# UoB-HPC/neutral

Measured on AMD Instinct MI355X. Metric: particle-steps/sec, higher is better.
Workload: dtype f64

## Files before the change

neutral_amd/csrc/neutral_abi.hip:

```cpp
#include "neutral_abi_state.h"

#include <utility>

using namespace neutral_abi;


namespace {

struct StageMs {
  double kernel = 0.0, sort = 0.0, stream = 0.0, collide = 0.0, exported = 0.0, exchange = 0.0;
};

struct Step {
  neutral::SolveArgs a = {};
  neutral::StepOptions options;
  bool tiled = false;
  bool decomposed = false;
  bool exchange = false;
  bool pass_export = false;
  bool checked = false;
  State::Store* shard = nullptr;
  neutral::StepCounters hc[2] = {};
  unsigned long long check[8] = {0};
  unsigned ctrl[16] = {0};
  unsigned long long words[kStepWords] = {0};
  int passes = 0;
  int attempts = 0;
  int same = 0;
  unsigned long long queue_total = 0;
  uint64_t local_nprocessed = 0;
  StageMs stage;
};

struct BatchSpec {
  neutral::TiledPlan plan;
  int first_pass;
  bool first_sort_timed;
  bool guarded;
  const neutral::SplitExport* split;
};

BatchSpec first_batch(const neutral::SplitExport* split) {
  BatchSpec spec = {};
  spec.plan.stream_passes = g.plan_passes > 0 ? g.plan_passes + 1 : 2;
  spec.plan.blocks_per_cu = -1;
  spec.first_pass = 0;
  spec.first_sort_timed = true;
  spec.guarded = true;
  spec.split = split;
  return spec;
}

BatchSpec later_batch(int stream_passes, int first_pass) {
  BatchSpec spec = {};
  spec.plan.stream_passes = stream_passes;
  spec.plan.blocks_per_cu = -1;
  spec.first_pass = first_pass;
  return spec;
}

void harvest(Step& s, bool with_sort) {
  StageMs& stage = s.stage;
  float ms = 0.0f;
  HIP_CHECK(hipEventElapsedTime(&ms, g.ev_start, g.ev_stop));
  stage.kernel += (double)ms;
  if (s.tiled) {
    if (with_sort) {
      HIP_CHECK(hipEventElapsedTime(&ms, g.ev_start, g.ev_sorted));
      stage.sort += (double)ms;
      HIP_CHECK(hipEventElapsedTime(&ms, g.ev_sorted, g.ev_streamed));
    } else {
      HIP_CHECK(hipEventElapsedTime(&ms, g.ev_start, g.ev_streamed));
    }
    stage.stream += (double)ms;
    HIP_CHECK(hipEventElapsedTime(&ms, g.ev_streamed, g.ev_collected));
    stage.sort += (double)ms;
    HIP_CHECK(hipEventElapsedTime(&ms, g.ev_collected, g.ev_stop));
    stage.collide += (double)ms;
  } else {
    stage.collide += (double)ms;
  }
  HIP_CHECK(hipEventElapsedTime(&ms, g.ev_stop, g.ev_exported));
  stage.exported += (double)ms;
  if (s.exchange) {
    HIP_CHECK(hipEventElapsedTime(&ms, g.ev_exchange_begins, g.ev_exchanged));
    stage.exchange += (double)ms;
  }
}

void export_records_by_id(const Step& s, const int* abort_flag) {
  const neutral::SolveArgs& a = s.a;
  HIP_CHECK(neutral::launch_export_records(
      g.tiled.rec_out, g.tiled.slot_of_id, a.p, a.nparticles, g.stream, abort_flag,
      a.export_skip_long_dead ? neutral::tiled_first_inactive(g.tiled) : nullptr, 0xFFFFFFFFu,
      nullptr, 0, a.export_skip_long_dead != 0));
}

void run_batch(Step& s, const BatchSpec& spec) {
  neutral::SolveArgs& a = s.a;
  HIP_CHECK(hipEventRecord(g.ev_start, g.stream));
  if (s.tiled) {
    HIP_CHECK(neutral::launch_solve_tiled(a, s.options, g.tiled, g.stream, spec.plan, spec.first_pass,
                                          spec.first_sort_timed ? g.ev_sorted : nullptr, g.ev_streamed,
                                          g.ev_collected, &s.passes, spec.split));
  } else {
    HIP_CHECK(neutral::launch_solve(a, s.options, g.variant, g.stream));
  }
  HIP_CHECK(hipEventRecord(g.ev_stop, g.stream));
  if (s.exchange) {
    exchange_step(a, s.tiled);
  } else {
    tallies_to_caller(a);
  }
  if (spec.split) {
    HIP_CHECK(neutral::launch_split_export(a, g.tiled, *spec.split, g.ev_collected));
    HIP_CHECK(hipStreamWaitEvent(g.stream, g.ev_split_done, 0));
  } else if (s.pass_export && !s.decomposed) {
    export_records_by_id(s, spec.guarded ? a.abort_flag : nullptr);
  }
  HIP_CHECK(hipEventRecord(g.ev_exported, g.stream));
  a.export_view = nullptr;
  g.tiled.mark_suspended = 0;

  if (s.exchange) {
    finish_exchange();
  }
  publish_results(s.tiled, s.exchange);
  wait_for_stream();
// ... 658 lines not shown
```

neutral_amd/csrc/neutral_abi_state.h:

```cpp
#ifndef NEUTRAL_AMD_ABI_STATE_H
#define NEUTRAL_AMD_ABI_STATE_H

#include "../../include/neutral_hip.h"

#include <hip/hip_runtime.h>

#include <math.h>
#include <stdio.h>
#include <stdlib.h>
#include <string.h>

#include "neutral_comm.h"
#include "neutral_kernels.h"

extern "C" {
#include "../host/comms.h"
}

extern "C" {
int get_key_value_parameter(const char* specifier, const char* filename, char* keys,
                            double* values, int* nkeys);
int within_tolerance(const double expected, const double result, const double tolerance);
}

// ... 81 lines not shown
  bool use_checked = false;
  const void* checked_density = nullptr;
  bool said_checked = false;
  unsigned short* d_index[2] = {nullptr, nullptr};
  unsigned short* d_index_fine = nullptr;
  hipEvent_t ev_start = nullptr;
  hipEvent_t ev_stop = nullptr;
  hipEvent_t ev_sorted = nullptr;
  hipEvent_t ev_streamed = nullptr;
  hipEvent_t ev_collected = nullptr;
  hipEvent_t ev_exported = nullptr;
  struct StepResults* h_results = nullptr;
  struct StepResults* d_results = nullptr;
  hipStream_t comm_stream = nullptr;
  hipEvent_t ev_exchanged = nullptr;
  hipEvent_t ev_exchange_begins = nullptr;
  TableView tables;
  neutral::TiledArgs tiled = {};
  const void* rec_owner = nullptr;
  neutral::ParticleView rec_owner_view = {};
  int rec_count = 0;
  bool rec_valid = false;
  bool carried_valid = false;
  bool soa_valid = true;
  int lazy_export = 0;
  int plan_passes = 0;
  unsigned final_from = 0xFFFFFFFFu;
  int host_syncs = 0;
  int exchange_rounds = 0;
  unsigned long long emigrants = 0;
  int host_collectives = 0;
  unsigned long long* d_words = nullptr;
  MeshTally tallies[kMeshTallies] = {{1, 0, false}, {1, 0, false}, {2, 0, true}, {2, 1, true}, {4, 1, true}};
  double* d_susp_current = nullptr;
  size_t susp_current_particles = 0;
  double roulette_cutoff = 0.0;
  double roulette_survival = 0.0;
  double* d_step_scalars = nullptr;
  double* spectrum_out = nullptr;
  int spectrum_ngroups = 0;
  int spectrum_box[4] = {0, 0, 0, 0};
  double spectrum_edges[neutral::kSpectrumMaxGroups + 1] = {};
  int auto_shard = 1;
  struct Store {
    const void* key;
    int count;
    uint64_t first;
    bool decomposed;
    int capacity;
    unsigned* keys;
  };
  bool domain_on = false;
  neutral::DomainGrid domain = {1, 1, 0, 0};
  double source_box[4] = {0.0, 0.0, 0.0, 0.0};
  bool source_box_set = false;
  unsigned* d_exchange = nullptr;
  neutral::ParticleRec* d_send = nullptr;
  neutral::ParticleRec* d_recv = nullptr;
  size_t send_capacity = 0;
  size_t recv_capacity = 0;
  unsigned* rec_owner_keys = nullptr;
  unsigned* d_free_slots = nullptr;
  size_t free_slots_capacity = 0;
  int free_count = 0;
  enum { kMaxStores = 64 };
  Store stores[kMaxStores] = {};
  int nstores = 0;
  double mesh_width = 1.0;
  double mesh_height = 1.0;
  const void* extent_edges = nullptr;
  double edge_dx = 0.0;
  double edge_dy = 0.0;
  int extent_nx = 0;
  int extent_ny = 0;
  int tiled_particles = 0;
  int tiled_tiles = 0;
  int tiled_chunks = 0;
  hipStream_t export_stream = nullptr;
  hipEvent_t ev_split_done = nullptr;
  neutral::ParticleView* d_export_view = nullptr;
  neutral::ParticleView h_export_view = {};
  bool export_view_uploaded = false;
  double suspended_share = -1.0;
  size_t susp_id_words = 0;
  neutral::LaunchTuning tuning = {};
  bool tuning_read = false;
  void* d_comb = nullptr;
  size_t comb_bytes = 0;
  int stream_queues = 0;
  size_t queue_places = 0;
  int queue_tiles = 0;
};

extern State g;

enum StepWord : int {
  kWordCounters = 0,
  kWordRequeued = 8,
  kWordCollidePasses = 9,
  kWordTurnedDown = 10,
  kWordMigrants = 11,
  kWordQueued = 12,
  kWordAborted = 13,
  kWordRanks = 14,
  kWordSteals = 15,
  kWordStealsRefused = 16,
  kWordWeightedWaves = 17,
  kWordRouletteKilled = 18,
  kWordRouletteSurvived = 19,
  kStepWords = 20,
};

void ensure_scratch();
void read_variant_env();
void wait_for_stream();
void* device_zalloc(size_t bytes);
void sync_soa();
void drop_records();
void ensure_tiled_workspace(int nx, int ny, int nparticles_now, int capacity);
void before_device_write(const void* dst, size_t bytes);
void refresh_table_view(const NeutralHipCrossSection* cs_s, const NeutralHipCrossSection* cs_a,
                        bool force, bool fast_arithmetic);
neutral::ParticleView view_of(const NeutralHipParticle* p);
const State::Store* find_store(const NeutralHipParticle* p);
State::Store* remember_store(const NeutralHipParticle* p, int count, uint64_t first);
void forget_store(const NeutralHipParticle* p);
inline bool flux_code_on() {
  return g.tallies[kTallyFlux].caller[0] != nullptr || g.tallies[kTallyCurrent].caller[0] != nullptr ||
         g.tallies[kTallyOutflow].caller[0] != nullptr;
}
neutral::StepOptions begin_step_scoring(neutral::SolveArgs& a, double* energy_tally, bool tiled,
                                        bool exchange);
void run_inject(const int nparticles, const int local_nx, const int local_ny, const int pad,
                const double left_off, const double bottom_off, const double width,
                const double height, const int x_off, const int y_off, const double dt,
                const double* edgex, const double* edgey, const double initial_energy,
                const NeutralHipParticle* particles);
void run_inject_filtered(State::Store* st, const int nparticles, const int local_nx,
                         const int local_ny, const int pad, const double left_off,
                         const double bottom_off, const double width, const double height,
                         const int x_off, const int y_off, const double dt, const double* edgex,
                         const double* edgey, const double initial_energy,
                         const NeutralHipParticle* particles);

void exchange_step(const neutral::SolveArgs& a, bool tiled);
void tallies_to_caller(const neutral::SolveArgs& a);
void finish_exchange();
void publish_results(bool tiled, bool with_words);
void fetch_results(neutral::StepCounters* hc, unsigned long long* check, unsigned* ctrl,
                   unsigned long long* words);
int exchange_particles(const neutral::SolveArgs& a, neutral::TiledArgs& t);

}
#endif
```

neutral_amd/csrc/neutral_abi_store.hip:

```cpp
#include "neutral_abi_state.h"

namespace neutral_abi {

State g;


void ensure_scratch() {
  int dev = 0;
  HIP_CHECK(hipGetDevice(&dev));
  if (g.scratch_device == dev) {
    return;
  }
  HIP_CHECK(hipMalloc((void**)&g.d_counters, 2 * sizeof(neutral::StepCounters)));
  HIP_CHECK(hipMalloc((void**)&g.d_check, 16 * sizeof(unsigned long long)));
  HIP_CHECK(hipMemset(g.d_check, 0, 16 * sizeof(unsigned long long)));
  HIP_CHECK(hipMalloc((void**)&g.d_exchange, sizeof(unsigned) * 200));
  HIP_CHECK(hipMalloc((void**)&g.d_words, sizeof(unsigned long long) * kStepWords));
  HIP_CHECK(hipMalloc((void**)&g.d_step_scalars, kStepScalars * sizeof(double)));
  g.tables.valid = false;
  HIP_CHECK(hipMalloc((void**)&g.d_index_fine,
                      sizeof(unsigned short) * (kMaxFineIndexBuckets + 1)));
  for (unsigned short*& d : g.d_index) {
    HIP_CHECK(hipMalloc((void**)&d, sizeof(unsigned short) * (kMaxIndexBuckets + 1)));
  }
  HIP_CHECK(hipEventCreate(&g.ev_start));
  HIP_CHECK(hipEventCreate(&g.ev_stop));
  HIP_CHECK(hipEventCreate(&g.ev_sorted));
  HIP_CHECK(hipEventCreate(&g.ev_streamed));
  HIP_CHECK(hipEventCreate(&g.ev_collected));
  HIP_CHECK(hipEventCreate(&g.ev_exported));
  HIP_CHECK(hipEventCreate(&g.ev_exchanged));
  HIP_CHECK(hipEventCreate(&g.ev_exchange_begins));
  HIP_CHECK(hipStreamCreateWithFlags(&g.comm_stream, hipStreamNonBlocking));
  {
    int least = 0, greatest = 0;
    HIP_CHECK(hipDeviceGetStreamPriorityRange(&least, &greatest));
    HIP_CHECK(hipStreamCreateWithPriority(&g.export_stream, hipStreamNonBlocking, least));
    HIP_CHECK(hipEventCreateWithFlags(&g.ev_split_done, hipEventDisableTiming));
    HIP_CHECK(hipMalloc((void**)&g.d_export_view, sizeof(neutral::ParticleView)));
    g.export_view_uploaded = false;
  }
  if (!g.h_results) {
    HIP_CHECK(hipHostMalloc((void**)&g.h_results, sizeof(StepResults), hipHostMallocMapped));
    memset(g.h_results, 0, sizeof(StepResults));
  }
  HIP_CHECK(hipHostGetDevicePointer((void**)&g.d_results, g.h_results, 0));
  g.scratch_device = dev;
}

void read_variant_env() {
  if (!g.variant_from_env_done) {
    g.variant_from_env_done = true;
    const char* v = getenv("NEUTRAL_HIP_VARIANT");
    if (v && *v) {
      const int iv = atoi(v);
      if (iv == NEUTRAL_HIP_VARIANT_OVER_PARTICLE || iv == NEUTRAL_HIP_VARIANT_EVENT_SORTED ||
          iv == NEUTRAL_HIP_VARIANT_TILED) {
        g.variant = iv;
      } else {
        fprintf(stderr, "libneutral_hip: ignoring NEUTRAL_HIP_VARIANT=%s\n", v);
      }
    }
  }
  if (!g.arithmetic_from_env_done) {
    g.arithmetic_from_env_done = true;
    const char* arith = getenv("NEUTRAL_HIP_ARITH");
    if (arith && strcmp(arith, "checked") == 0) {
      g.arithmetic = NEUTRAL_HIP_ARITH_CHECKED;
    }
  }
}

void wait_for_stream() {
  HIP_CHECK(hipStreamSynchronize(g.stream));
  g.host_syncs++;
}

void* device_zalloc(size_t bytes) {
  void* p = nullptr;
  HIP_CHECK(hipMalloc(&p, bytes ? bytes : 1));
  HIP_CHECK(hipMemsetAsync(p, 0, bytes ? bytes : 1, g.stream));
  HIP_CHECK(hipStreamSynchronize(g.stream));
  return p;
}

neutral::CsIndex build_index(const double* d_keys, int n, unsigned short* d_start,
                             int first_shift = 44 ,
                             int max_buckets = kMaxIndexBuckets) {
  neutral::CsIndex ix = {nullptr, 0, 0, 0};
  if (n < 2 || n > 65535) {
    return ix;
  }
  double ends[2];
  HIP_CHECK(hipMemcpyAsync(&ends[0], d_keys, sizeof(double), hipMemcpyDeviceToHost, g.stream));
  HIP_CHECK(hipMemcpyAsync(&ends[1], d_keys + (n - 1), sizeof(double), hipMemcpyDeviceToHost,
                           g.stream));
  wait_for_stream();
  if (!(ends[0] > 0.0) || !(ends[1] > ends[0])) {
    return ix;
  }
  long long lo_bits, hi_bits;
  memcpy(&lo_bits, &ends[0], sizeof(lo_bits));
  memcpy(&hi_bits, &ends[1], sizeof(hi_bits));
  int shift = first_shift;
  while (((hi_bits >> shift) - (lo_bits >> shift) + 1) > max_buckets) {
    shift++;
  }
  ix.shift = shift;
  ix.base = lo_bits >> shift;
  ix.nbuckets = (int)((hi_bits >> shift) - ix.base + 1);
  HIP_CHECK(neutral::launch_build_cs_index(d_keys, n, ix.shift, ix.base, ix.nbuckets, d_start,
                                           g.stream));
  ix.start = d_start;
  return ix;
}

void sync_soa() {
  if (!g.soa_valid && g.rec_valid && g.rec_owner) {
    if (g.rec_owner_keys) {
      HIP_CHECK(neutral::launch_export_by_slot(g.tiled.rec_in, g.rec_owner_view, g.rec_owner_keys,
                                               g.rec_count, g.stream));
    } else {
      HIP_CHECK(neutral::launch_export_records(g.tiled.rec_in, g.tiled.slot_of_id,
// ... 856 lines not shown
```

neutral_amd/csrc/neutral_kernels.h:

```cpp
#ifndef NEUTRAL_AMD_KERNELS_H
#define NEUTRAL_AMD_KERNELS_H

#include <hip/hip_runtime.h>
#include <stdint.h>

namespace neutral {

struct ParticleView {
  double* x;
  double* y;
  double* omega_x;
  double* omega_y;
  double* energy;
  double* weight;
  double* dt_to_census;
  double* mfp_to_collision;
  int* cellx;
  int* celly;
  int* dead;
};

struct alignas(16) ParticleRec {
  double x, y, dt_to_census, mfp_to_collision;
  int cellx, celly;
// ... 116 lines not shown
  CarriedStart* carried;
  int steal_min;
  StealWork* steal;
  int steal_delay;
  int occupancy_rows;
  int share_weight;
  int weighted_share_min;
  int compute_units;
  int export_skip_long_dead;
  const ParticleView* export_view;
  int decomposed;
  unsigned* emigrants;
  const int* abort_flag;
};

struct TiledArgs {
  ParticleRec* rec_in;
  ParticleRec* rec_out;
  unsigned* info_in;
  unsigned* info_out;
  unsigned* id_in;
  unsigned* id_out;
  unsigned* slot_of_id;
  CarriedStart* carried_in;
  CarriedStart* carried_out;
  int carried;
  int sort_end;
  int mirror_end;
  int slots_by_id;
  unsigned* order;
  unsigned* tile_count;
  unsigned* tile_offset;
  unsigned* tile_cursor;
  uint4* chunks;
  unsigned* collide_queue;
  unsigned* susp_ids;
  int mark_suspended;
  SuspendExtra* susp;
  double* susp_track;
  StealWork* steal;
  unsigned* queue_entries;
  unsigned* queue_tail;
  unsigned* queue_head;
  unsigned queue_capacity;
  const unsigned short* fine_index;
  int fine_index_n;
  long long fine_index_base;
  int fine_index_shift;
  int* edges_computed;
  unsigned char* tile_uniform;
  unsigned* ctrl;
  int chunk_particles;
  int refill_min;
  int stream_repeat;
  int pass;
  int allow_migrate;
  double cells_per_x;
  double cells_per_y;
  int tile_shift;
  int window_min_particles;
  int tiles_x;
  int tiles_y;
  int ntiles;
  int reach_classes;
  int nsort;
  int max_chunks;
};

struct LaunchTuning {
  int steal_min;
  int share_weight;
  int weighted_share_min;
  int steal_delay;
  int max_blocks;
  int compute_units;
};
LaunchTuning launch_tuning_from_env();

struct DomainGrid {
  int px, py;
  int bx, by;
};

struct TiledPlan {
  int stream_passes;
  int blocks_per_cu;
};

enum Variant {
  kVariantOverParticle = 0,
  kVariantEventSorted = 1,
  kVariantTiled = 2,
};

hipError_t launch_inject(const InjectArgs& a, hipStream_t stream);
hipError_t launch_inject_filtered(const InjectArgs& a, unsigned* keys, unsigned* count,
                                  hipStream_t stream);
constexpr int kSpectrumMaxGroups = 64;
struct SpectrumParams {
  double* buffer;
  int ngroups;
  int x0, y0;
  unsigned width, height;
  double edges[kSpectrumMaxGroups + 1];
};
struct CurrentParams {
  double* jx;
  double* jy;
  double* susp;
};
struct StepOptions {
  double* collision_tallies = nullptr;
  double roulette_cutoff = 0.0;
  double roulette_survival = 0.0;
  SpectrumParams spectrum = {};
  CurrentParams current = {nullptr, nullptr, nullptr};
  double* outflow = nullptr;
};
enum Score : unsigned {
  kScoreCollisions = 1,
  kScoreRoulette = 2,
  kScoreSpectrum = 4,
  kScoreCurrent = 8,
  kScoreOutflow = 16,
};
constexpr int kScoreBits = 5;
constexpr unsigned kScoresOfStreaming = kScoreSpectrum | kScoreCurrent | kScoreOutflow;
inline unsigned scores_of(const StepOptions& o) {
  return (o.collision_tallies ? kScoreCollisions : 0u) | (o.roulette_cutoff > 0.0 ? kScoreRoulette : 0u) |
         (o.spectrum.ngroups > 0 ? kScoreSpectrum : 0u) | (o.current.jx ? kScoreCurrent : 0u) |
         (o.outflow ? kScoreOutflow : 0u);
}
constexpr bool scores_instantiated(bool flux, unsigned scores) {
  return flux || !(scores & (kScoreCurrent | kScoreOutflow));
}
hipError_t set_step_options(const StepOptions& o, hipStream_t stream);
hipError_t set_step_options_tiled(const StepOptions& o, hipStream_t stream);
hipError_t launch_solve(const SolveArgs& a, const StepOptions& o, int variant, hipStream_t stream);
hipError_t launch_unphysical_values(const double* v, long long n, unsigned long long* out,
                                    hipStream_t stream);
hipError_t launch_tables_check(const double* ks, const double* vs, int ns, const double* ka,
                               const double* va, int na, unsigned long long expect_hash_s,
                               unsigned long long expect_hash_a, int expect_same,
                               int fast_arithmetic, unsigned long long* out4,
                               hipStream_t stream);


size_t tiled_lds_bytes(const SolveArgs& a, const StepOptions& o, const TiledArgs& t);
hipError_t launch_import_records(const ParticleView& p, ParticleRec* rec, unsigned* info,
                                 unsigned* slot_of_id, unsigned* ids, int tiles_x, int tile_shift,
                                 int x_off, int y_off, int n, hipStream_t stream);
hipError_t launch_refresh_micro(const SolveArgs& a, const TiledArgs& t, hipStream_t stream);
bool tiled_uses_carried(const SolveArgs& a, const TiledArgs& t);
hipError_t launch_export_records(const ParticleRec* rec, const unsigned* slot_of_id,
                                 const ParticleView& p, int n, hipStream_t stream,
                                 const int* abort_flag = nullptr,
                                 const unsigned* first_inactive = nullptr,
                                 unsigned final_from = 0xFFFFFFFFu,
                                 const unsigned* skip_ids = nullptr, int max_blocks = 0,
                                 bool partial_ok = false);
struct SplitExport {
  bool on;
  hipStream_t side;
  hipEvent_t done;
  ParticleView p;
  int skip_long_dead;
};
// ... 65 lines not shown
```

neutral_amd/csrc/neutral_tiled.hip:

```cpp
#include <cstdlib>
#include <cstring>
#include <type_traits>

#include "neutral_kernels.h"

#include "neutral_device.h"
#include "neutral_history.h"
#include "neutral_step_options.h"
#include "neutral_wave.h"

namespace neutral {

#ifndef NEUTRAL_STREAM_BLOCK
#define NEUTRAL_STREAM_BLOCK 1024
#endif
constexpr int kStreamBlock = NEUTRAL_STREAM_BLOCK;
constexpr int kChunkParticlesMax = 32768;
constexpr int kChunkParticlesMin = 1024;
constexpr int kStreamRefillMin = 56;
constexpr int kStreamRepeat = 64;
constexpr int kStreamRepeatOnePass = 128;
#ifdef NEUTRAL_NO_CARRIED_START
constexpr bool kCarriedStart = false;
#else
// ... 54 lines not shown
__device__ __forceinline__ bool step_is_broken(const SolveArgs& a) {
  return a.counters->aborted != 0u;
}

__global__ __launch_bounds__(kSortBlock) void tile_count_kernel(SolveArgs a, TiledArgs t) {
  extern __shared__ unsigned s_bins[];
  if (pass_is_empty(t) || (t.pass > 0 && step_is_broken(a))) {
    return;
  }
  const int nbins = t.nsort + 1;
  const bool in_lds = nbins <= kSortLdsBins;
  if (in_lds) {
    for (int b = threadIdx.x; b < nbins; b += kSortBlock) {
      s_bins[b] = 0;
    }
    __syncthreads();
  }
  const unsigned* info = sort_summaries(t);
  const long long base = (long long)blockIdx.x * kSortSegment;
#pragma unroll 4
  for (int k = 0; k < kSortItems; ++k) {
    const long long i = base + (long long)k * kSortBlock + threadIdx.x;
    const unsigned b = (i < t.sort_end) ? sort_bucket(t, info[i]) : kNoBucket;
    if (in_lds) {
      if (b != kNoBucket) {
        atomicAdd(&s_bins[b], 1u);
      }
    } else {
      const bool is_dead = (b == (unsigned)t.nsort);
      const unsigned long long m_dead = __ballot(is_dead);
      if (b != kNoBucket && !is_dead) {
        atomicAdd(&t.tile_count[b], 1u);
      }
      if (m_dead != 0 && (threadIdx.x & 63) == (unsigned)__ffsll((long long)m_dead) - 1u) {
        atomicAdd(&t.tile_count[t.nsort], (unsigned)__popcll(m_dead));
      }
    }
  }
  if (in_lds) {
    __syncthreads();
    for (int b = threadIdx.x; b < nbins; b += kSortBlock) {
      const unsigned c = s_bins[b];
      if (c) {
        atomicAdd(&t.tile_count[b], c);
      }
    }
  }
}

__global__ __launch_bounds__(1024) void tile_scan_kernel(TiledArgs t) {
  __shared__ unsigned s_part[1024];
  const int tid = threadIdx.x;
  const int n = t.nsort + 2;
  const int per = (n + 1023) / 1024;
  const int lo = (tid * per < n) ? tid * per : n;
  const int hi = (lo + per < n) ? lo + per : n;
  unsigned sum = 0;
  for (int i = lo; i < hi; ++i) {
    sum += (i <= t.nsort) ? t.tile_count[i] : 0u;
  }
  s_part[tid] = sum;
  __syncthreads();
  for (int off = 1; off < 1024; off <<= 1) {
    const unsigned c0 = (tid >= off) ? s_part[tid - off] : 0;
    __syncthreads();
    s_part[tid] += c0;
    __syncthreads();
  }
  if (tid == 0) {
    t.ctrl[kCtrlWindowed] = 0;
  }
  unsigned run = s_part[tid] - sum;
  for (int i = lo; i < hi; ++i) {
    const unsigned c = (i <= t.nsort) ? t.tile_count[i] : 0u;
    t.tile_offset[i] = run;
    t.tile_cursor[i] = run;
    if (i <= t.nsort) {
      t.tile_count[i] = 0;
    }
    run += c;
  }
}

__device__ __forceinline__ void draw_for_slot(const SolveArgs& a, const TiledArgs& t, long long slot) {
  t.carried_in[slot].minus_log_rn0 = draw_first_flight(a.pid_base + (uint64_t)t.id_in[slot], a.master_key);
}

__global__ __launch_bounds__(kSortBlock) void tile_scatter_kernel(SolveArgs a, TiledArgs t) {
  extern __shared__ unsigned s_bins[];
  if (pass_is_empty(t) || (t.pass > 0 && step_is_broken(a))) {
    return;
  }
  const bool draws = t.pass == 0 && t.carried != 0;
  const int nbins = t.nsort + 1;
  const bool in_lds = nbins <= kSortLdsBins;
  unsigned* s_rank = s_bins;
  unsigned* s_base = s_bins + nbins;
  const unsigned* info = sort_summaries(t);
  const long long base = (long long)blockIdx.x * kSortSegment;
  unsigned bucket[kSortItems];
#pragma unroll
  for (int k = 0; k < kSortItems; ++k) {
    const long long i = base + (long long)k * kSortBlock + threadIdx.x;
    bucket[k] = (i < t.sort_end) ? sort_bucket(t, info[i]) : kNoBucket;
  }
  if (!in_lds) {
#pragma unroll
    for (int k = 0; k < kSortItems; ++k) {
      const bool is_dead = (bucket[k] == (unsigned)t.nsort);
      const unsigned long long m_dead = __ballot(is_dead);
      unsigned dead_base = 0;
      if (m_dead != 0) {
        const unsigned leader = (unsigned)__ffsll((long long)m_dead) - 1u;
        if ((threadIdx.x & 63) == leader) {
          dead_base = atomicAdd(&t.tile_cursor[t.nsort], (unsigned)__popcll(m_dead));
        }
        dead_base = __shfl(dead_base, (int)leader, 64);
      }
      if (bucket[k] != kNoBucket) {
        const unsigned pos = is_dead ? dead_base + (unsigned)lane_rank(m_dead)
                                     : atomicAdd(&t.tile_cursor[bucket[k]], 1u);
        t.order[pos] = (unsigned)(base + (long long)k * kSortBlock + threadIdx.x);
        if (draws && !is_dead) {
          draw_for_slot(a, t, base + (long long)k * kSortBlock + threadIdx.x);
        }
      }
    }
    return;
  }
  for (int b = threadIdx.x; b < nbins; b += kSortBlock) {
    s_rank[b] = 0;
  }
  __syncthreads();
#pragma unroll
  for (int k = 0; k < kSortItems; ++k) {
    if (bucket[k] != kNoBucket) {
      atomicAdd(&s_rank[bucket[k]], 1u);
    }
  }
  __syncthreads();
  for (int b = threadIdx.x; b < nbins; b += kSortBlock) {
    const unsigned c = s_rank[b];
    if (c) {
      s_base[b] = atomicAdd(&t.tile_cursor[b], c);
      s_rank[b] = 0;
    }
  }
  __syncthreads();
#pragma unroll
  for (int k = 0; k < kSortItems; ++k) {
    if (bucket[k] != kNoBucket) {
      const unsigned pos = s_base[bucket[k]] + atomicAdd(&s_rank[bucket[k]], 1u);
      t.order[pos] = (unsigned)(base + (long long)k * kSortBlock + threadIdx.x);
    }
  }
  if (draws) {
#pragma unroll 1
    for (int k = 0; k < kSortItems; ++k) {
      if (bucket[k] != kNoBucket && bucket[k] != (unsigned)t.nsort) {
        draw_for_slot(a, t, base + (long long)k * kSortBlock + threadIdx.x);
      }
    }
  }
}

__global__ __launch_bounds__(kSortBlock) void copy_inactive_kernel(SolveArgs a, TiledArgs t) {
  if (a.abort_flag && *a.abort_flag) {
    return;
  }
  const unsigned first_inactive = t.tile_offset[t.nsort];
  const unsigned ncarried = (unsigned)t.sort_end - first_inactive;
  const unsigned total = ncarried + (unsigned)(t.mirror_end - t.sort_end);
  for (unsigned u = blockIdx.x * kSortBlock + threadIdx.x; u < total; u += gridDim.x * kSortBlock) {
  if (u < ncarried) {
    const unsigned j = first_inactive + u;
    const unsigned src = t.order[j];
    const ParticleRec r = t.rec_in[src];
    t.rec_out[j] = r;
    t.info_out[j] = t.info_in[src];
    if (a.decomposed) {
      t.id_out[j] = t.id_in[src];
    } else {
      t.slot_of_id[r.id] = j;
    }
  } else {
    const unsigned m = (unsigned)t.sort_end + (u - ncarried);
    if (m < (unsigned)t.mirror_end) {
      t.rec_out[m] = t.rec_in[m];
      t.info_out[m] = t.info_in[m];
    }
  }
  }
}

__global__ __launch_bounds__(kSortBlock) void collect_suspended_kernel(SolveArgs a, TiledArgs t,
                                                                       const unsigned* info) {
  __shared__ unsigned s_count[kSortItems][kSortBlock / 64];
  __shared__ unsigned s_base;
  if (step_is_broken(a)) {
    return;
  }
  const long long base = (long long)blockIdx.x * kSortSegment;
  const int wave = threadIdx.x >> 6;
  unsigned mine = 0;
#pragma unroll
  for (int k = 0; k < kSortItems; ++k) {
    const long long i = base + (long long)k * kSortBlock + threadIdx.x;
    const bool susp = i < t.sort_end && summary_state(info[i]) == kRecCollide;
    const unsigned long long m = __ballot(susp);
    mine |= susp ? (1u << k) : 0u;
    if ((threadIdx.x & 63) == 0) {
      s_count[k][wave] = (unsigned)__popcll(m);
    }
  }
  __syncthreads();
  if (threadIdx.x == 0) {
    unsigned total = 0;
    for (int k = 0; k < kSortItems; ++k) {
      for (int w = 0; w < kSortBlock / 64; ++w) {
        const unsigned c = s_count[k][w];
        s_count[k][w] = total;
        total += c;
      }
    }
    s_base = total ? atomicAdd(&t.ctrl[kCtrlCollideCount], total) : 0u;
  }
  __syncthreads();
  if (mine) {
#pragma unroll
    for (int k = 0; k < kSortItems; ++k) {
      const bool susp = ((mine >> k) & 1u) != 0;
      const unsigned long long m = __ballot(susp);
      if (susp) {
        const unsigned slot = (unsigned)(base + (long long)k * kSortBlock + threadIdx.x);
        t.collide_queue[s_base + s_count[k][wave] + (unsigned)lane_rank(m)] = slot;
        if (t.mark_suspended) {
          const unsigned id = t.rec_out[slot].id;
          atomicOr(&t.susp_ids[id >> 5], 1u << (id & 31u));
        }
      }
    }
  }
}

__global__ __launch_bounds__(kSortBlock) void import_records_kernel(ParticleView p, ParticleRec* rec,
                                                                    unsigned* info,
// ... 1125 lines not shown
         kStreamLdsControlBytes + sizeof(double) * 2 * (size_t)o.spectrum.ngroups;
}

int tiled_chunk_particles(int nparticles, int compute_units) {
  long long c = (long long)nparticles / ((long long)compute_units * 6);
  if (c > kChunkParticlesMax) c = kChunkParticlesMax;
  if (c < kChunkParticlesMin) c = kChunkParticlesMin;
  return (int)c;
}

int tiled_tile_shift(int nx, int ny, int nparticles, bool with_flux) {
  const int largest = with_flux ? 6 : 7;
  const char* force = getenv("NEUTRAL_TILE_CELLS");
  if (force) {
    const int cells = atoi(force);
    for (int shift = 4; shift <= largest; ++shift) {
      if (cells == (1 << shift)) {
        return shift;
      }
    }
  }
  const double density = (double)nparticles / ((double)nx * (double)ny);
  const int shift = (density >= 8.0) ? 4 : (density >= 2.0) ? 5 : (density >= 0.5) ? 6 : 7;
  return shift < largest ? shift : largest;
}

int tiled_window_min_particles(int tile_shift) {
  const char* force = getenv("NEUTRAL_WINDOW_MIN_PARTICLES");
  if (force) {
    return atoi(force);
  }
  return (tile_shift >= 7) ? 64 : (2048 >> (tile_shift - 4));
}

void tiled_geometry(int nx, int ny, int nparticles, int tile_shift, int* tiles_x, int* tiles_y,
                    int* max_chunks) {
  const int tile = 1 << tile_shift;
  *tiles_x = (nx + tile - 1) / tile;
  *tiles_y = (ny + tile - 1) / tile;
  *max_chunks = (*tiles_x) * (*tiles_y) + nparticles / kChunkParticlesMin + 1;
}

hipError_t launch_import_records(const ParticleView& p, ParticleRec* rec, unsigned* info,
                                 unsigned* slot_of_id, unsigned* ids, int tiles_x, int tile_shift,
                                 int x_off, int y_off, int n, hipStream_t stream) {
  if (n > 0) {
    hipLaunchKernelGGL(import_records_kernel, dim3((n + kSortBlock - 1) / kSortBlock),
                       dim3(kSortBlock), 0, stream, p, rec, info, slot_of_id, ids, tiles_x, tile_shift,
                       x_off, y_off, n);
  }
  return hipGetLastError();
}

hipError_t launch_refresh_micro(const SolveArgs& a, const TiledArgs& t, hipStream_t stream) {
  if (t.sort_end > 0) {
    hipLaunchKernelGGL(refresh_micro_kernel, dim3((t.sort_end + kSortBlock - 1) / kSortBlock),
                       dim3(kSortBlock), 0, stream, a, t);
  }
  return hipGetLastError();
}

bool tiled_uses_carried(const SolveArgs& a, const TiledArgs& t) {
  return kCarriedStart && a.same_tables && !a.decomposed && !t.queue_entries && t.carried_in &&
         t.carried_out;
}

hipError_t launch_export_records(const ParticleRec* rec, const unsigned* slot_of_id,
                                 const ParticleView& p, int n, hipStream_t stream,
                                 const int* abort_flag, const unsigned* first_inactive,
                                 unsigned final_from, const unsigned* skip_ids, int max_blocks,
                                 bool partial_ok) {
  if (n > 0) {
    int grid = (n + kSortBlock - 1) / kSortBlock;
    grid = (max_blocks > 0 && grid > max_blocks) ? max_blocks : grid;
    hipLaunchKernelGGL(export_records_kernel, dim3(grid), dim3(kSortBlock), 0, stream, rec,
                       slot_of_id, p, n, abort_flag, first_inactive, final_from, skip_ids, partial_ok ? 1 : 0);
  }
  return hipGetLastError();
}

const unsigned* tiled_first_inactive(const TiledArgs& t) { return &t.ctrl[kCtrlFirstInactive]; }

static hipError_t enqueue_stream_pass(const SolveArgs& a, const StepOptions& o, TiledArgs& t, int pass,
                                      int cus, size_t lds, hipStream_t stream, hipEvent_t after_sort) {
  t.pass = pass;
  t.allow_migrate = (pass + 1 < kMaxStreamPasses) ? 1 : 0;
  const int grid_n = (a.nparticles + kSortBlock - 1) / kSortBlock;
  const int grid_seg = t.sort_end > 0 ? (t.sort_end + kSortSegment - 1) / kSortSegment : 1;
  const int nbins = t.nsort + 1;
  const size_t lds_bins = (nbins <= kSortLdsBins) ? sizeof(unsigned) * (size_t)nbins : 0;
  hipLaunchKernelGGL(tile_count_kernel, dim3(grid_seg), dim3(kSortBlock), lds_bins, stream, a, t);
  hipLaunchKernelGGL(tile_scan_kernel, dim3(1), dim3(1024), 0, stream, t);
  hipLaunchKernelGGL(tile_scatter_kernel, dim3(grid_seg), dim3(kSortBlock), 2 * lds_bins, stream, a,
                     t);
  hipLaunchKernelGGL(tile_chunks_kernel, dim3(1), dim3(1024), 0, stream, t);
  if (pass == 0) {
    hipLaunchKernelGGL(copy_inactive_kernel, dim3(grid_n < 8192 ? grid_n : 8192), dim3(kSortBlock), 0, stream,
                       a, t);
    if (after_sort) {
      (void)hipEventRecord(after_sort, stream);
    }
  }
  if (t.queue_entries) {
    hipLaunchKernelGGL(queue_reset_kernel, dim3(t.ntiles), dim3(kSortBlock), 0, stream, t);
  }
  auto launch = [&](auto kernel) {
    (void)hipFuncSetAttribute((const void*)kernel, hipFuncAttributeMaxDynamicSharedMemorySize,
                              (int)lds);
    hipLaunchKernelGGL(kernel, dim3(cus), dim3(kStreamBlock), lds, stream, a, t);
  };
  const unsigned pick = (t.queue_entries ? 16u : 0u) | (a.checked ? 8u : 0u) | (a.decomposed ? 4u : 0u) |
                        (a.flux_tally ? 2u : 0u) | (a.same_tables ? 1u : 0u);
  return with_constant<5 + kScoreBits>(pick << kScoreBits | (scores_of(o) & kScoresOfStreaming), [&](auto chosen) {
    constexpr unsigned kPick = decltype(chosen)::value >> kScoreBits;
    constexpr unsigned kScores = decltype(chosen)::value & ((1u << kScoreBits) - 1u);
    constexpr bool kFlux = (kPick & 2u) != 0;
    if constexpr ((kScores & ~kScoresOfStreaming) == 0 && scores_instantiated(kFlux, kScores)) {
      launch(stream_kernel<(kPick & 1u) != 0, kFlux, (kPick & 4u) != 0, (kPick & 8u) != 0, (kPick & 16u) != 0, kScores>);
      return hipGetLastError();
    } else {
      return hipErrorInvalidValue;
    }
  });
}

hipError_t launch_solve_tiled(const SolveArgs& a, const StepOptions& o, TiledArgs& t, hipStream_t stream,
                              const TiledPlan& plan, int first_pass, hipEvent_t after_sort,
                              hipEvent_t after_stream, hipEvent_t after_collect,
                              int* passes_enqueued, const SplitExport* split) {
  if (passes_enqueued) {
    *passes_enqueued = first_pass;
  }
  if (a.nparticles <= 0) {
    if (after_sort && first_pass == 0) (void)hipEventRecord(after_sort, stream);
    if (after_stream) (void)hipEventRecord(after_stream, stream);
    if (after_collect) (void)hipEventRecord(after_collect, stream);
    return hipSuccess;
  }
  if (a.decomposed || t.sort_end > a.nparticles || t.mirror_end < t.sort_end) {
    t.sort_end = a.nparticles;
    t.mirror_end = a.nparticles;
  }
  const int cus = a.compute_units > 0 ? a.compute_units : 256;
  t.chunk_particles = tiled_chunk_particles(a.nparticles, cus);
  t.refill_min = kStreamRefillMin;
  t.stream_repeat = (plan.stream_passes <= 2) ? kStreamRepeatOnePass : kStreamRepeat;
  t.carried = tiled_uses_carried(a, t) ? 1 : 0;
  const size_t lds = tiled_lds_bytes(a, o, t);
  (void)hipFuncSetAttribute((const void*)tile_scatter_kernel,
                            hipFuncAttributeMaxDynamicSharedMemorySize,
                            (int)(2 * sizeof(unsigned) * kSortLdsBins));

  if (first_pass == 0 && t.edges_computed) {
    hipLaunchKernelGGL(edges_check_kernel, dim3(1), dim3(1024), 0, stream, a, t);
  }
  if (first_pass == 0 && t.tile_uniform && a.pad == 0) {
    hipLaunchKernelGGL(tile_uniform_kernel, dim3(t.ntiles), dim3(kSortBlock), 0, stream, a, t,
                       stream_window_cells(a, o, t));
  } else if (first_pass == 0 && t.tile_uniform) {
    (void)hipMemsetAsync(t.tile_uniform, 0, (size_t)t.ntiles, stream);
  }
  int pass = first_pass;
  for (int k = 0; k < plan.stream_passes && pass < kMaxStreamPasses; ++k, ++pass) {
    const hipError_t err = enqueue_stream_pass(a, o, t, pass, cus, lds, stream, after_sort);
    if (err != hipSuccess) {
      return err;
    }
  }
  if (passes_enqueued) {
    *passes_enqueued = pass;
  }
  if (after_stream) {
    (void)hipEventRecord(after_stream, stream);
  }

  hipLaunchKernelGGL(collect_suspended_kernel,
                     dim3(t.sort_end > 0 ? (t.sort_end + kSortSegment - 1) / kSortSegment : 1),
                     dim3(kSortBlock), 0, stream, a, t, t.info_out);
  if (after_collect) {
    (void)hipEventRecord(after_collect, stream);
  }
  SolveArgs c = a;
  c.blocks_per_cu = plan.blocks_per_cu;
  c.counters = a.counters + 1;
  c.queue = t.collide_queue;
  c.queue_len = &t.ctrl[kCtrlCollideCount];
  c.rec = t.rec_out;
  c.slot_info = t.info_out;
  c.tiles_x = t.tiles_x;
  c.tile_shift = t.tile_shift;
  c.susp = t.susp;
  c.susp_track = t.susp_track;
  c.carried = t.carried ? t.carried_out : nullptr;
  c.steal = t.steal;
  c.emigrants = &t.ctrl[kCtrlEmigrants];
  if (t.fine_index && c.same_tables) {
    c.scatter_index = t.fine_index;
    c.scatter_index_n = t.fine_index_n;
    c.scatter_index_base = t.fine_index_base;
    c.index_shift = t.fine_index_shift;
  }
  return launch_solve(c, o, kVariantEventSorted, stream);
}

hipError_t launch_split_export(const SolveArgs& a, const TiledArgs& t, const SplitExport& split,
                               hipEvent_t after_collect) {
  (void)hipStreamWaitEvent(split.side, after_collect, 0);
  (void)launch_export_records(t.rec_out, t.slot_of_id, split.p, a.nparticles, split.side, a.abort_flag,
                              split.skip_long_dead ? &t.ctrl[kCtrlFirstInactive] : nullptr, 0xFFFFFFFFu,
                              t.susp_ids, 0, split.skip_long_dead != 0);
  (void)hipEventRecord(split.done, split.side);
  return hipGetLastError();
}


}
```

Measured before the change: 150.6 billion.

## Move first-flight draws and inactive copy to a side stream overlapping sort

Takes the first-flight random draws out of the scatter kernel and puts them in a standalone kernel. That kernel runs on a new side stream, concurrently with the tile count, scan and scatter kernels. The copy-inactive kernel also moves to the side stream after the scatter and overlaps with tile_chunks and the first stream kernel, and the main stream waits on events before and after the stream kernel. The aim is to shorten the serial sort prelude, at the cost of extra event records, cross-stream waits and an extra kernel launch. The stream kernel may now run while copy_inactive is still writing, which is a correctness risk if they touch the same data.

```diff
diff --git a/neutral_amd/csrc/neutral_abi.hip b/neutral_amd/csrc/neutral_abi.hip
--- a/neutral_amd/csrc/neutral_abi.hip
+++ b/neutral_amd/csrc/neutral_abi.hip
@@ -44,6 +44,7 @@
   BatchSpec spec = {};
   spec.plan.stream_passes = g.plan_passes > 0 ? g.plan_passes + 1 : 2;
   spec.plan.blocks_per_cu = -1;
+  spec.plan.side = &g.prelude;
   spec.first_pass = 0;
   spec.first_sort_timed = true;
   spec.guarded = true;
diff --git a/neutral_amd/csrc/neutral_abi_state.h b/neutral_amd/csrc/neutral_abi_state.h
--- a/neutral_amd/csrc/neutral_abi_state.h
+++ b/neutral_amd/csrc/neutral_abi_state.h
@@ -187,6 +187,7 @@
   neutral::ParticleView h_export_view = {};
   bool export_view_uploaded = false;
   double suspended_share = -1.0;
+  neutral::PreludeSide prelude = {};
   size_t susp_id_words = 0;
   neutral::LaunchTuning tuning = {};
   bool tuning_read = false;
diff --git a/neutral_amd/csrc/neutral_abi_store.hip b/neutral_amd/csrc/neutral_abi_store.hip
--- a/neutral_amd/csrc/neutral_abi_store.hip
+++ b/neutral_amd/csrc/neutral_abi_store.hip
@@ -39,6 +39,11 @@
     HIP_CHECK(hipEventCreateWithFlags(&g.ev_split_done, hipEventDisableTiming));
     HIP_CHECK(hipMalloc((void**)&g.d_export_view, sizeof(neutral::ParticleView)));
     g.export_view_uploaded = false;
+    HIP_CHECK(hipStreamCreateWithFlags(&g.prelude.stream, hipStreamNonBlocking));
+    HIP_CHECK(hipEventCreateWithFlags(&g.prelude.forked, hipEventDisableTiming));
+    HIP_CHECK(hipEventCreateWithFlags(&g.prelude.drawn, hipEventDisableTiming));
+    HIP_CHECK(hipEventCreateWithFlags(&g.prelude.placed, hipEventDisableTiming));
+    HIP_CHECK(hipEventCreateWithFlags(&g.prelude.carried_over, hipEventDisableTiming));
   }
   if (!g.h_results) {
     HIP_CHECK(hipHostMalloc((void**)&g.h_results, sizeof(StepResults), hipHostMallocMapped));
diff --git a/neutral_amd/csrc/neutral_kernels.h b/neutral_amd/csrc/neutral_kernels.h
--- a/neutral_amd/csrc/neutral_kernels.h
+++ b/neutral_amd/csrc/neutral_kernels.h
@@ -222,7 +222,16 @@
   int bx, by;
 };
 
+struct PreludeSide {
+  hipStream_t stream;
+  hipEvent_t forked;
+  hipEvent_t drawn;
+  hipEvent_t placed;
+  hipEvent_t carried_over;
+};
+
 struct TiledPlan {
+  const PreludeSide* side;
   int stream_passes;
   int blocks_per_cu;
 };
diff --git a/neutral_amd/csrc/neutral_tiled.hip b/neutral_amd/csrc/neutral_tiled.hip
--- a/neutral_amd/csrc/neutral_tiled.hip
+++ b/neutral_amd/csrc/neutral_tiled.hip
@@ -160,16 +160,11 @@
   }
 }
 
-__device__ __forceinline__ void draw_for_slot(const SolveArgs& a, const TiledArgs& t, long long slot) {
-  t.carried_in[slot].minus_log_rn0 = draw_first_flight(a.pid_base + (uint64_t)t.id_in[slot], a.master_key);
-}
-
 __global__ __launch_bounds__(kSortBlock) void tile_scatter_kernel(SolveArgs a, TiledArgs t) {
   extern __shared__ unsigned s_bins[];
   if (pass_is_empty(t) || (t.pass > 0 && step_is_broken(a))) {
     return;
   }
-  const bool draws = t.pass == 0 && t.carried != 0;
   const int nbins = t.nsort + 1;
   const bool in_lds = nbins <= kSortLdsBins;
   unsigned* s_rank = s_bins;
@@ -199,9 +194,6 @@
         const unsigned pos = is_dead ? dead_base + (unsigned)lane_rank(m_dead)
                                      : atomicAdd(&t.tile_cursor[bucket[k]], 1u);
         t.order[pos] = (unsigned)(base + (long long)k * kSortBlock + threadIdx.x);
-        if (draws && !is_dead) {
-          draw_for_slot(a, t, base + (long long)k * kSortBlock + threadIdx.x);
-        }
       }
     }
     return;
@@ -232,14 +224,18 @@
       t.order[pos] = (unsigned)(base + (long long)k * kSortBlock + threadIdx.x);
     }
   }
-  if (draws) {
-#pragma unroll 1
-    for (int k = 0; k < kSortItems; ++k) {
-      if (bucket[k] != kNoBucket && bucket[k] != (unsigned)t.nsort) {
-        draw_for_slot(a, t, base + (long long)k * kSortBlock + threadIdx.x);
-      }
-    }
-  }
+}
+
+__global__ __launch_bounds__(kSortBlock) void first_draws_kernel(SolveArgs a, TiledArgs t) {
+  const long long slot = (long long)blockIdx.x * kSortBlock + threadIdx.x;
+  if (slot >= t.sort_end) {
+    return;
+  }
+  const int state = summary_state(t.info_in[slot]);
+  if (state == kRecGone || state == kRecDead) {
+    return;
+  }
+  t.carried_in[slot].minus_log_rn0 = draw_first_flight(a.pid_base + (uint64_t)t.id_in[slot], a.master_key);
 }
 
 __global__ __launch_bounds__(kSortBlock) void copy_inactive_kernel(SolveArgs a, TiledArgs t) {
@@ -1531,21 +1527,47 @@
 const unsigned* tiled_first_inactive(const TiledArgs& t) { return &t.ctrl[kCtrlFirstInactive]; }
 
 static hipError_t enqueue_stream_pass(const SolveArgs& a, const StepOptions& o, TiledArgs& t, int pass,
-                                      int cus, size_t lds, hipStream_t stream, hipEvent_t after_sort) {
+                                      int cus, size_t lds, hipStream_t stream, hipEvent_t after_sort,
+                                      const PreludeSide* side) {
   t.pass = pass;
   t.allow_migrate = (pass + 1 < kMaxStreamPasses) ? 1 : 0;
   const int grid_n = (a.nparticles + kSortBlock - 1) / kSortBlock;
   const int grid_seg = t.sort_end > 0 ? (t.sort_end + kSortSegment - 1) / kSortSegment : 1;
   const int nbins = t.nsort + 1;
   const size_t lds_bins = (nbins <= kSortLdsBins) ? sizeof(unsigned) * (size_t)nbins : 0;
+  const bool draws = pass == 0 && t.carried != 0 && t.sort_end > 0;
+  hipStream_t beside = (pass == 0 && side) ? side->stream : stream;
+  if (pass == 0 && side) {
+    (void)hipEventRecord(side->forked, stream);
+    (void)hipStreamWaitEvent(side->stream, side->forked, 0);
+  }
+  if (draws) {
+    hipLaunchKernelGGL(first_draws_kernel, dim3((t.sort_end + kSortBlock - 1) / kSortBlock), dim3(kSortBlock),
+                       0, beside, a, t);
+  }
+  if (pass == 0 && side) {
+    (void)hipEventRecord(side->drawn, side->stream);
+  }
   hipLaunchKernelGGL(tile_count_kernel, dim3(grid_seg), dim3(kSortBlock), lds_bins, stream, a, t);
   hipLaunchKernelGGL(tile_scan_kernel, dim3(1), dim3(1024), 0, stream, t);
   hipLaunchKernelGGL(tile_scatter_kernel, dim3(grid_seg), dim3(kSortBlock), 2 * lds_bins, stream, a,
                      t);
+  if (pass == 0) {
+    if (side) {
+      (void)hipEventRecord(side->placed, stream);
+      (void)hipStreamWaitEvent(side->stream, side->placed, 0);
+    }
+    hipLaunchKernelGGL(copy_inactive_kernel, dim3(grid_n < 8192 ? grid_n : 8192), dim3(kSortBlock), 0, beside,
+                       a, t);
+    if (side) {
+      (void)hipEventRecord(side->carried_over, side->stream);
+    }
+  }
   hipLaunchKernelGGL(tile_chunks_kernel, dim3(1), dim3(1024), 0, stream, t);
   if (pass == 0) {
-    hipLaunchKernelGGL(copy_inactive_kernel, dim3(grid_n < 8192 ? grid_n : 8192), dim3(kSortBlock), 0, stream,
-                       a, t);
+    if (side) {
+      (void)hipStreamWaitEvent(stream, side->drawn, 0);
+    }
     if (after_sort) {
       (void)hipEventRecord(after_sort, stream);
     }
@@ -1560,7 +1582,7 @@
   };
   const unsigned pick = (t.queue_entries ? 16u : 0u) | (a.checked ? 8u : 0u) | (a.decomposed ? 4u : 0u) |
                         (a.flux_tally ? 2u : 0u) | (a.same_tables ? 1u : 0u);
-  return with_constant<5 + kScoreBits>(pick << kScoreBits | (scores_of(o) & kScoresOfStreaming), [&](auto chosen) {
+  const hipError_t err = with_constant<5 + kScoreBits>(pick << kScoreBits | (scores_of(o) & kScoresOfStreaming), [&](auto chosen) {
     constexpr unsigned kPick = decltype(chosen)::value >> kScoreBits;
     constexpr unsigned kScores = decltype(chosen)::value & ((1u << kScoreBits) - 1u);
     constexpr bool kFlux = (kPick & 2u) != 0;
@@ -1571,6 +1593,10 @@
       return hipErrorInvalidValue;
     }
   });
+  if (pass == 0 && side) {
+    (void)hipStreamWaitEvent(stream, side->carried_over, 0);
+  }
+  return err;
 }
 
 hipError_t launch_solve_tiled(const SolveArgs& a, const StepOptions& o, TiledArgs& t, hipStream_t stream,
@@ -1611,7 +1637,7 @@
   }
   int pass = first_pass;
   for (int k = 0; k < plan.stream_passes && pass < kMaxStreamPasses; ++k, ++pass) {
-    const hipError_t err = enqueue_stream_pass(a, o, t, pass, cus, lds, stream, after_sort);
+    const hipError_t err = enqueue_stream_pass(a, o, t, pass, cus, lds, stream, after_sort, plan.side);
     if (err != hipSuccess) {
       return err;
     }
```

Result: no change. 148.8 billion (median of 2 runs) (-1.2%).
